# LiuZhu-CV/PAIF

Hardware: AMD Instinct MI355X
Metric: fused image-pairs/sec at 480x640 bs=8 per GPU (fusion-net forward) (higher is better)
Workload: dtype f16 (IEEE fp16 maps and conv weights, one fp16 MFMA per product, f32 accumulate; stems, guided filter and the last map fp32)

## Files before the change

paif_amd/csrc/conv_dma.h:

```cpp
#pragma once
#include <hip/hip_runtime.h>

namespace paif_conv_dma {

struct Args {
  const void* src[3];
  const void* res[3];
  const void* wpk;
  const float* scale;
  const float* shift;
  const float* prelu;
  void* out;
  float alpha;
  int nsrc, nres, act, kh;
  int cout;
  int B, H, W, reverse;
  float* cpool;
  int f16;
  int dil;
  int in_relu;
  int out_f32;
};

bool eligible(int nsrc, int nres, int B, int H, int W, float alpha);
bool eligible16(int nsrc, int nres, int B, int H, int W, float alpha);
bool eligible7(int nsrc, int nres, int B, int H, int W, float alpha);
bool eligible_d2(int nsrc, int nres, int B, int H, int W, float alpha);
bool can_cpool(int nsrc, int nres, int kh, int cout, int dil);
int launch(const Args& a, hipStream_t st);

bool eligible_1x1(int nsrc, int nres, int B, int H, int W);
int launch_1x1(const Args& a, hipStream_t st);

bool eligible_rows(int nsrc, int nres, int in_relu, int cpool, int f16, int out_f32, int B, int H, int W);
int launch_rows(const Args& a, hipStream_t st);

}
```

paif_amd/csrc/conv_mfma.hip:

```cpp
#include <stdlib.h>

#include "conv_dma.h"
#include "paif_common.h"
#include <type_traits>

#ifndef PAIF_UB_HOOKS
#define PAIF_UB_HOOKS 3
#endif
#ifndef PAIF_UB
#define PAIF_UB 11
#endif

namespace {

typedef float f32x16 __attribute__((ext_vector_type(16)));

#ifndef PAIF_TH
#define PAIF_TH 8
#endif
constexpr int TH = PAIF_TH;
constexpr int TW = 32;
constexpr int NTHREADS = 256;
constexpr int SEGS_PER_WAVE = TH / 4;

// ... 1292 lines not shown
  } else {
    const int t = tid - 4 * 64;
    const int q = t & 7, px = t >> 3;
    const float4 sc = *reinterpret_cast<const float4*>((a.scale ? a.scale : k_ones) + 4 * q);
    const float4 sh = *reinterpret_cast<const float4*>((a.shift ? a.shift : k_zeros) + 4 * q);
    const float slope = *(a.act == 1 ? a.prelu : k_zeros);
    const int nres = a.res[0] ? (a.res[1] ? (a.res[2] ? 3 : 2) : 1) : 0;
    const unsigned lane_off = (unsigned)px * 32u + 4u * (unsigned)q;
    auto run = [&](auto nres_c) {
      constexpr int NR = decltype(nres_c)::value;
      float4 r[NR > 0 ? NR : 1][8];
      auto request = [&](int i) {
        int b, y0, x0;
        tile_of(min(i, cnt - 1), b, y0, x0);
        const size_t base = ((size_t)(b * a.H + y0) * a.W + x0) * 32;
        const unsigned lo = x0 + px < a.W ? lane_off : 0u;
#pragma unroll
        for (int k = 0; k < NR; ++k)
#pragma unroll
          for (int j = 0; j < 8; ++j) {
            const int yy = min(y0 + j, a.H - 1) - y0;
            r[k][j] = paif::ldq_nt<BFR>(a.res[k], base + (size_t)yy * a.W * 32 + lo);
          }
      };
      if (cnt > 0) request(0);
      int s2 = 0, i2 = 0;
      for (int g = 0; g <= S + 1; ++g) {
        if (g >= 2) {
          if (s2 == nsrc - 1) {
            int b, y0, x0;
            tile_of(i2, b, y0, x0);
            float4 o[8];
#pragma unroll
            for (int j = 0; j < 8; ++j) o[j] = *reinterpret_cast<const float4*>(outbuf + (j * 32 + px) * 32 + 4 * q);
            const size_t base = ((size_t)(b * a.H + y0) * a.W + x0) * 32;
            const bool colok = x0 + px < a.W;
#pragma unroll
            for (int j = 0; j < 8; ++j) {
              float4 v = o[j];
              v.x = v.x * sc.x + sh.x; v.y = v.y * sc.y + sh.y; v.z = v.z * sc.z + sh.z; v.w = v.w * sc.w + sh.w;
              if (a.act == 1) {
                v.x = paif::prelu_f(v.x, slope); v.y = paif::prelu_f(v.y, slope);
                v.z = paif::prelu_f(v.z, slope); v.w = paif::prelu_f(v.w, slope);
              } else if (a.act == 2) {
                v.x = fmaxf(v.x, 0.f); v.y = fmaxf(v.y, 0.f); v.z = fmaxf(v.z, 0.f); v.w = fmaxf(v.w, 0.f);
              }
              v.x *= a.alpha; v.y *= a.alpha; v.z *= a.alpha; v.w *= a.alpha;
#pragma unroll
              for (int k = 0; k < NR; ++k) { v.x += r[k][j].x; v.y += r[k][j].y; v.z += r[k][j].z; v.w += r[k][j].w; }
              if (colok && y0 + j < a.H)
                paif::stq_nt<BFO>(a.out, base + (size_t)j * a.W * 32 + lane_off, v);
              if (a.cpool) {
                float mx = fmaxf(fmaxf(v.x, v.y), fmaxf(v.z, v.w)), sm = (v.x + v.y) + (v.z + v.w);
                paif::pix8_max_sum(mx, sm);
                if (colok && y0 + j < a.H && q == 0)
                  *reinterpret_cast<float2*>(a.cpool + ((base + (size_t)j * a.W * 32) >> 5) * 4 + (size_t)px * 4) = make_float2(mx, sm * (1.0f / 32.0f));
              }
            }
            if (NR > 0) request(i2 + 1);
          }
          if (++s2 == nsrc) { s2 = 0; ++i2; }
        }
        lds_barrier();
        lds_barrier();
      }
    };
    if (nres == 0) run(std::integral_constant<int, 0>{});
    else if (nres == 1) run(std::integral_constant<int, 1>{});
    else if (nres == 2) run(std::integral_constant<int, 2>{});
    else run(std::integral_constant<int, 3>{});
  }
}

template <int KH, int DIL, int ST = 0>
__global__ __launch_bounds__(WS_THREADS, 1) void conv_bf16x3_ws(ConvArgs a, int ntiles) { conv_ws_body<KH, DIL, ST, false>(a, ntiles); }
template <int KH, int DIL, int ST = 0>
__global__ __launch_bounds__(WS_THREADS, 1) void conv_bf16x3_wsr(ConvArgs a, int ntiles) { conv_ws_body<KH, DIL, ST, true>(a, ntiles); }

template <int KH, int DIL, int ST = 0>
int launch_bf16x3_ws(const ConvArgs& a, hipStream_t st) {
  constexpr int P = DIL * (KH - 1) / 2;
  constexpr size_t lds_bytes = 2 * (size_t)(TH + 2 * P) * (TW + 2 * P) * 144 + 8 * 32 * 32 * 4;
  static_assert(lds_bytes <= 160 * 1024, "two tile buffers + the parked tile do not fit LDS");
  static bool raised = false;
  constexpr bool HAS_RELU = KH == 3 && DIL == 2 && paif::st_in(ST) != 0 && paif::st_low(ST) != 7;
  if (!raised) {
    hipError_t e = hipFuncSetAttribute(reinterpret_cast<const void*>(&conv_bf16x3_ws<KH, DIL, ST>),
                                       hipFuncAttributeMaxDynamicSharedMemorySize, (int)lds_bytes);
    if constexpr (HAS_RELU) {
      if (e == hipSuccess)
        e = hipFuncSetAttribute(reinterpret_cast<const void*>(&conv_bf16x3_wsr<KH, DIL, ST>), hipFuncAttributeMaxDynamicSharedMemorySize,
                                (int)lds_bytes);
    }
    if (e != hipSuccess) {
      paif::set_error("conv2d(bf16x3 ws): cannot raise dynamic LDS to %zu: %s", lds_bytes, hipGetErrorString(e));
      return (int)e;
    }
    raised = true;
  }
  if (a.in_act == 2) {
    if constexpr (HAS_RELU) {
      hipLaunchKernelGGL((conv_bf16x3_wsr<KH, DIL, ST>), dim3(256), dim3(WS_THREADS), lds_bytes, st, a, a.nblk);
      PAIF_LAUNCH_CHECK("conv2d(bf16x3 wsr)");
      return 0;
    }
    paif::set_error("conv2d(bf16x3 ws): input ReLU is built for the bf16-stored dilation-2 3x3 only");
    return PAIF_ENOSUP;
  }
  hipLaunchKernelGGL((conv_bf16x3_ws<KH, DIL, ST>), dim3(256), dim3(WS_THREADS), lds_bytes, st, a, a.nblk);
  PAIF_LAUNCH_CHECK("conv2d(bf16x3 ws)");
  return 0;
}

static inline bool ws_enabled() {
  static const bool on = [] {
    const char* e = getenv("PAIF_CONV_WS");
    return !(e && e[0] == '0');
  }();
  return on;
}
static inline bool st_h16(const ConvArgs& a) { return a.st == 1 || a.st == 3; }
static inline bool st_is_f16(const ConvArgs& a) { return a.st >= 3; }
static inline bool ws_eligible(const ConvArgs& a) {
  return ws_enabled() && a.nblk >= 1024 && !a.pool_partial && a.cout == 32 && (a.in_act == 0 || (a.in_act == 2 && st_h16(a))) &&
         (size_t)a.H * a.W * 128 < ((size_t)1 << 32);
}

static inline bool res_eligible(const ConvArgs& a) {
  static const bool on = [] {
    const char* e = getenv("PAIF_CONV_RES");
    return !(e && e[0] == '0');
  }();
  static const int ms_res = [] {
    const char* e = getenv("PAIF_CONV_RES_NSRC");
    return e ? atoi(e) : 1;
  }();
  return on && !st_is_f16(a) && (a.nsrc == 1 || (a.wl0 && a.st == 1 && a.in_act == 0 && a.nsrc <= ms_res)) && a.nblk >= 2048 && a.cout == 32 && a.in_act <= 2 && (PAIF_RES_ROWS == 8 || !a.pool_partial) &&
         (size_t)a.B * a.H * a.W * 128 < ((size_t)1 << 31);
}

static inline bool needs_hooks(const ConvArgs& a) { return a.in_act >= 3 || a.aux_out || a.epi_dact; }

static inline bool takes_ws(const ConvArgs& a, int kh, int dil) {
#if PAIF_TH == 8
  if (needs_hooks(a) || kh > 3 || !ws_eligible(a)) return false;
  if (a.st == 4) return dil == 2 && a.nsrc == 1 && a.in_act == 0;
  if (kh == 1) return !a.res[0] && a.in_act == 0;
  return dil == 2 && a.nsrc == 1 && st_h16(a);
#else
  return false;
#endif
}

enum ConvVariant { CV_PLAIN, CV_HOOKS, CV_WS, CV_RES, CV_MS, CV_DMA, CV_ROWS };
static inline int res_count(const ConvArgs& a) { return a.res[0] ? (a.res[1] ? (a.res[2] ? 3 : 2) : 1) : 0; }
static inline ConvVariant bf16x3_variant(const ConvArgs& a, int kh, int dil) {
  if (needs_hooks(a)) return CV_HOOKS;
  if (dil == 1 && st_h16(a) && a.wl0 && a.in_act == 0 && !a.pool_partial &&
      ((kh == 3 && a.cout == 32 && paif_conv_dma::eligible(a.nsrc, res_count(a), a.B, a.H, a.W, a.alpha)) ||
       (kh == 3 && a.cout == 16 && paif_conv_dma::eligible16(a.nsrc, res_count(a), a.B, a.H, a.W, a.alpha)) ||
       (kh == 7 && a.cout == 32 && paif_conv_dma::eligible7(a.nsrc, res_count(a), a.B, a.H, a.W, a.alpha))))
    return CV_DMA;
  if (kh == 3 && dil == 2 && (st_h16(a) || a.st == 4) && a.wl0 && a.in_act == 0 && !a.pool_partial && !a.cpool && a.cout == 32 &&
      paif_conv_dma::eligible_rows(a.nsrc, res_count(a), 0, 0, st_is_f16(a) ? 1 : 0, a.st == 4 ? 1 : 0, a.B, a.H, a.W))
    return CV_ROWS;
  if (kh == 3 && dil == 2 && st_h16(a) && a.wl0 && a.in_act == 2 && !a.pool_partial && a.cout == 32 &&
      paif_conv_dma::eligible_d2(a.nsrc, res_count(a), a.B, a.H, a.W, a.alpha))
    return CV_DMA;
  if (kh == 1 && dil == 1 && st_h16(a) && a.wl0 && a.in_act == 0 && !a.pool_partial && a.cout == 32 && ws_eligible(a) &&
      paif_conv_dma::eligible_1x1(a.nsrc, res_count(a), a.B, a.H, a.W))
    return CV_DMA;
  if (takes_ws(a, kh, dil)) return CV_WS;
  if (kh == 3 && dil == 1 && !st_is_f16(a)) {
    if (res_eligible(a)) return CV_RES;
    if (ms_enabled() && a.nsrc >= 2 && a.cout == 32 && a.in_act == 0 && !a.pool_partial &&
        (size_t)a.B * a.H * a.W * 128 < ((size_t)1 << 32))
      return CV_MS;
  }
  return CV_PLAIN;
}

static inline bool variant_can_cpool(const ConvArgs& a, int kh, int dil) {
  if (a.cout != 32 || needs_hooks(a)) return false;
  if (bf16x3_variant(a, kh, dil) == CV_DMA) return paif_conv_dma::can_cpool(a.nsrc, res_count(a), kh, a.cout, dil);
  return true;
}

template <int KH, int DIL, int ST>
int launch_bf16x3_st(const ConvArgs& a, hipStream_t st) {
  const ConvVariant cv = bf16x3_variant(a, KH, DIL);
  switch (cv) {
    case CV_ROWS:
    case CV_DMA: {
      paif_conv_dma::Args d{};
      for (int s = 0; s < 3; ++s) { d.src[s] = a.src[s]; d.res[s] = a.res[s]; }
      d.wpk = a.wpk; d.scale = a.scale; d.shift = a.shift; d.prelu = a.prelu; d.out = a.out; d.alpha = a.alpha;
      d.nsrc = a.nsrc; d.nres = res_count(a); d.act = a.act; d.B = a.B; d.H = a.H; d.W = a.W; d.reverse = a.reverse; d.kh = KH; d.cout = a.cout;
      d.f16 = paif::st_f16(ST) ? 1 : 0;
      d.cpool = a.cpool;
      d.dil = DIL; d.in_relu = a.in_act == 2 ? 1 : 0;
      d.out_f32 = paif::st_out(ST) == 0 ? 1 : 0;
      return cv == CV_ROWS ? paif_conv_dma::launch_rows(d, st) : paif_conv_dma::launch(d, st);
    }
    case CV_HOOKS:
      if constexpr (ST == 0) return launch_bf16x3_h<KH, DIL, true>(a, st);
      paif::set_error("conv2d: the gradient hooks (in_act >= 3, aux_out, epi_dact) are built for fp32 storage only");
      return PAIF_ENOSUP;
    case CV_WS:
#if PAIF_TH == 8
      if constexpr (KH <= 3) return launch_bf16x3_ws<KH, DIL, ST>(a, st);
#endif
      break;
    case CV_RES:
      if constexpr (KH == 3 && DIL == 1 && !paif::st_f16(ST)) {
        if constexpr (ST == 4) {
          if (a.nsrc == 2) return launch_bf16x3_res<3, 1, 2, ST>(a, st);
          if (a.nsrc == 3) return launch_bf16x3_res<3, 1, 3, ST>(a, st);
        }
        return launch_bf16x3_res<3, 1, 1, ST>(a, st);
      }
      break;
    case CV_MS:
      if constexpr (KH == 3 && DIL == 1 && !paif::st_f16(ST)) return a.nsrc == 2 ? launch_bf16x3_ms<3, 1, 2, ST>(a, st) : launch_bf16x3_ms<3, 1, 3, ST>(a, st);
      break;
    default: break;
  }
  return launch_bf16x3_h<KH, DIL, false, ST>(a, st);
}

static inline int kernel_st(const ConvArgs& a) {
  if (a.st == 4) return 15;
  const int st = a.st == 3 ? 1 : a.st;
  const int base = st == 1 ? (a.in_act == 1 ? 3 : 1) : st;
  const int code = (a.wl0 && base) ? base + 3 : base;
  return a.st >= 3 ? code + 8 : code;
}

template <int KH, int DIL>
int launch_bf16x6(const ConvArgs& a, hipStream_t st) {
  if (a.st != 0) {
    paif::set_error("conv2d: precision bf16x6 is built for fp32-stored maps");
    return PAIF_ENOSUP;
  }
  return needs_hooks(a) ? launch_bf16x3_h<KH, DIL, true, 0, 3>(a, st) : launch_bf16x3_h<KH, DIL, false, 0, 3>(a, st);
}

template <int KH, int DIL>
int launch_f16x3(const ConvArgs& a, hipStream_t st) {
  if (a.st != 0) {
    paif::set_error("conv2d: precision f16x3 is built for fp32-stored maps");
    return PAIF_ENOSUP;
  }
  return needs_hooks(a) ? launch_bf16x3_h<KH, DIL, true, 0, 2, 1>(a, st) : launch_bf16x3_h<KH, DIL, false, 0, 2, 1>(a, st);
}

template <int KH, int DIL>
int launch_bf16x3(const ConvArgs& a, hipStream_t st) {
  const int code = kernel_st(a);
  if (code == 0) return launch_bf16x3_st<KH, DIL, 0>(a, st);
  if constexpr ((KH == 1 || KH == 3 || KH == 7) && (DIL == 1 || (KH == 3 && DIL == 2))) {
    switch (code) {
      case 1: return launch_bf16x3_st<KH, DIL, 1>(a, st);
      case 3: return launch_bf16x3_st<KH, DIL, 3>(a, st);
      case 4: return launch_bf16x3_st<KH, DIL, 4>(a, st);
      case 6: return launch_bf16x3_st<KH, DIL, 6>(a, st);
      default: break;
    }
    if constexpr (KH == 1) {
      if (code == 2) return launch_bf16x3_st<KH, DIL, 2>(a, st);
      if (code == 5) return launch_bf16x3_st<KH, DIL, 5>(a, st);
    }
    switch (code) {
      case 12: return launch_bf16x3_st<KH, DIL, 12>(a, st);
      case 14: return launch_bf16x3_st<KH, DIL, 14>(a, st);
      default: break;
    }
    if constexpr (KH == 1) {
      if (code == 9) return launch_bf16x3_st<KH, DIL, 9>(a, st);
    }
    if constexpr (KH == 3 && DIL == 2) {
      if (code == 15) return launch_bf16x3_st<KH, DIL, 15>(a, st);
    }
  }
  paif::set_error("conv2d: storage %d is not built for the %dx%d dilation-%d kernel", a.st, KH, KH, DIL);
  return PAIF_ENOSUP;
}

__global__ void pack_weight_bf16x3_kernel(const float* __restrict__ w, unsigned short* __restrict__ wpk, int cout, int nsrc,
                                          int kh) {
  const int ntap = kh * kh;
  const int total = nsrc * ntap * 2 * 2 * 64 * 8;
  for (int idx = blockIdx.x * blockDim.x + threadIdx.x; idx < total; idx += gridDim.x * blockDim.x) {
    const int j = idx & 7, lane = (idx >> 3) & 63, part = (idx >> 9) & 1, ks = (idx >> 10) & 1;
    int rest = idx >> 11;
    const int tap = rest % ntap;
    const int s = rest / ntap;
    const int n = lane & 31, hh = lane >> 5;
    const int c = s * 32 + 16 * ks + 8 * hh + j;
    const float v = (n < cout) ? w[((size_t)n * (nsrc * 32) + c) * ntap + tap] : 0.f;
    const __bf16 hi = (__bf16)v;
    const __bf16 out = part == 0 ? hi : (__bf16)(v - (float)hi);
    wpk[idx] = __builtin_bit_cast(unsigned short, out);
  }
}

__global__ void compose_dw_pw_kernel(const float* __restrict__ dw, const float* __restrict__ pw, float* __restrict__ out, int cout,
                                     int cin, int ntap) {
  const int total = cout * cin * ntap;
  for (int idx = blockIdx.x * blockDim.x + threadIdx.x; idx < total; idx += gridDim.x * blockDim.x) {
    const int tap = idx % ntap, ci = (idx / ntap) % cin, co = idx / (ntap * cin);
    out[idx] = pw[co * cin + ci] * dw[ci * ntap + tap];
  }
}

__global__ void compose_pw_conv_kernel(const float* __restrict__ pw, const float* __restrict__ w, float* __restrict__ out, int cout, int cmid,
                                       int cin, int ntap) {
  const int total = cout * cin * ntap;
  for (int idx = blockIdx.x * blockDim.x + threadIdx.x; idx < total; idx += gridDim.x * blockDim.x) {
    const int rest = idx % (cin * ntap), co = idx / (cin * ntap);
    double acc = 0.0;
    for (int m = 0; m < cmid; ++m) acc = fma((double)pw[co * cmid + m], (double)w[(size_t)m * cin * ntap + rest], acc);
    out[idx] = (float)acc;
  }
}

__device__ __forceinline__ unsigned short bf16x6_piece(float v, int part) {
  const __bf16 hi = (__bf16)v;
  const float r1 = v - (float)hi;
  const __bf16 mid = (__bf16)r1;
  const __bf16 out = part == 0 ? hi : (part == 1 ? mid : (__bf16)(r1 - (float)mid));
  return __builtin_bit_cast(unsigned short, out);
}
__global__ void pack_weight_bf16x6_kernel(const float* __restrict__ w, unsigned short* __restrict__ wpk, int cout, int nsrc, int kh) {
  const int ntap = kh * kh;
  const int total = nsrc * ntap * 2 * 3 * 64 * 8;
  for (int idx = blockIdx.x * blockDim.x + threadIdx.x; idx < total; idx += gridDim.x * blockDim.x) {
    const int j = idx & 7, lane = (idx >> 3) & 63;
    int rest = idx >> 9;
    const int part = rest % 3; rest /= 3;
    const int ks = rest & 1; rest >>= 1;
    const int tap = rest % ntap;
    const int s = rest / ntap;
    const int n = lane & 31, hh = lane >> 5;
    const int c = s * 32 + 16 * ks + 8 * hh + j;
    const float v = (n < cout) ? w[((size_t)n * (nsrc * 32) + c) * ntap + tap] : 0.f;
    wpk[idx] = bf16x6_piece(v, part);
  }
}
__global__ void pack_decomp1x1_bf16x6_kernel(const float* __restrict__ w, unsigned short* __restrict__ wpk) {
  const int total = 3 * 2 * 3 * 64 * 8;
  for (int idx = blockIdx.x * blockDim.x + threadIdx.x; idx < total; idx += gridDim.x * blockDim.x) {
    const int j = idx & 7, lane = (idx >> 3) & 63;
    int rest = idx >> 9;
    const int part = rest % 3; rest /= 3;
// ... 45 lines not shown
    const float v = (n < cout) ? w[((size_t)n * (nsrc * 32) + c) * ntap + tap] : 0.f;
    wpk[idx] = f16x2_piece(v, part);
  }
}
__global__ void pack_decomp1x1_hf_f16x2_kernel(const float* __restrict__ w, unsigned short* __restrict__ wpk) {
  const int total = 3 * 2 * 2 * 64 * 8;
  for (int idx = blockIdx.x * blockDim.x + threadIdx.x; idx < total; idx += gridDim.x * blockDim.x) {
    const int j = idx & 7, lane = (idx >> 3) & 63, part = (idx >> 9) & 1, ks = (idx >> 10) & 1, s = idx >> 11;
    const int n = lane & 31, hh = lane >> 5;
    const int c = 16 * ks + 8 * hh + j;
    const float* wn = w + n * 128;
    float v;
    if (s == 0) v = wn[c] + wn[32 + c];
    else if (s == 1) v = wn[64 + c] - wn[c];
    else v = wn[96 + c] - wn[32 + c];
    wpk[idx] = f16x2_piece(v, part);
  }
}

template <int KH, int DIL, int CIN, bool HOOKS>
int launch_h(const ConvArgs& a, hipStream_t st) {
  constexpr int P = DIL * (KH - 1) / 2;
  constexpr size_t tile_bytes = (size_t)(TH + 2 * P) * (TW + 2 * P) * (CIN + 4) * 4;
  constexpr size_t epi_bytes = (size_t)TH * 32 * 32 * 4;
  constexpr size_t lds_bytes = tile_bytes > epi_bytes ? tile_bytes : epi_bytes;
  static_assert(lds_bytes <= 160 * 1024, "tile does not fit LDS");
  if (lds_bytes > 64 * 1024) {
    hipError_t e = hipFuncSetAttribute(reinterpret_cast<const void*>(&conv_mfma_f32<KH, DIL, CIN, HOOKS>),
                                       hipFuncAttributeMaxDynamicSharedMemorySize, (int)lds_bytes);
    if (e != hipSuccess) {
      paif::set_error("conv2d: cannot raise dynamic LDS to %zu: %s", lds_bytes, hipGetErrorString(e));
      return (int)e;
    }
  }
  hipLaunchKernelGGL((conv_mfma_f32<KH, DIL, CIN, HOOKS>), dim3(a.nblk), dim3(NTHREADS), lds_bytes, st, a);
  PAIF_LAUNCH_CHECK("conv2d");
  return 0;
}

template <int KH, int DIL, int CIN>
int launch(const ConvArgs& a, hipStream_t st) {
  return needs_hooks(a) ? launch_h<KH, DIL, CIN, true>(a, st) : launch_h<KH, DIL, CIN, false>(a, st);
}

__global__ void pack_weight_kernel(const float* __restrict__ w, float* __restrict__ wpk, int cout, int nsrc, int cin,
                                   int kh) {
  const int ntap = kh * kh, no = cin / 8;
  const int total = nsrc * ntap * no * 256;
  for (int idx = blockIdx.x * blockDim.x + threadIdx.x; idx < total; idx += gridDim.x * blockDim.x) {
    const int i = idx & 3, lane = (idx >> 2) & 63;
    int rest = idx >> 8;
    const int o = rest % no; rest /= no;
    const int tap = rest % ntap;
    const int s = rest / ntap;
    const int n = lane & 31, h = lane >> 5;
    const int c = s * cin + 8 * o + 4 * h + i;
    wpk[idx] = (n < cout) ? w[((size_t)n * (nsrc * cin) + c) * ntap + tap] : 0.f;
  }
}

__global__ void pack_decomp1x1_kernel(const float* __restrict__ w, float* __restrict__ wpk) {
  const int total = 3 * 4 * 256;
  for (int idx = blockIdx.x * blockDim.x + threadIdx.x; idx < total; idx += gridDim.x * blockDim.x) {
    const int i = idx & 3, lane = (idx >> 2) & 63;
    const int o = (idx >> 8) & 3, s = idx >> 10;
    const int n = lane & 31, h = lane >> 5;
    const int c = 8 * o + 4 * h + i;
    const float* wn = w + n * 128;
    float v;
    if (s == 0) v = wn[64 + c] + wn[96 + c];
    else if (s == 1) v = wn[c] - wn[64 + c];
    else v = wn[32 + c] - wn[96 + c];
    wpk[idx] = v;
  }
}

__global__ void bn_fold_kernel(const float* g, const float* bta, const float* mean, const float* var, float eps,
                               float* scale, float* shift, int C) {
  const int c = blockIdx.x * blockDim.x + threadIdx.x;
  if (c < C) {
    const float s = g[c] / sqrtf(var[c] + eps);
    scale[c] = s;
    shift[c] = bta[c] - mean[c] * s;
  }
}

}

extern "C" {

int paif_conv2d_blocks(int B, int H, int W) { return B * ((H + TH - 1) / TH) * ((W + TW - 1) / TW); }

size_t paif_conv_wpk_floats(int nsrc, int cin, int kh) { return (size_t)nsrc * kh * kh * (cin / 8) * 256; }

int paif_conv2d_is_persistent(const paif_conv_desc* d, int B, int H, int W) {
  if (!d || (d->precision != PAIF_CONV_BF16X3 && d->precision != PAIF_CONV_BF16 && d->precision != PAIF_CONV_F16 && d->precision != PAIF_CONV_F16X2) ||
      d->cin != 32 || B <= 0 || H <= 0 || W <= 0)
    return 0;
  ConvArgs a{};
  for (int s = 0; s < 3; ++s) a.res[s] = d->res[s];
  a.pool_partial = d->pool_partial; a.nsrc = d->nsrc; a.in_act = d->in_act; a.cout = d->cout;
  a.aux_out = d->aux_out; a.epi_dact = d->epi_dact; a.st = d->storage;
  a.H = H; a.W = W;
  a.nblk = B * ((W + TW - 1) / TW) * ((H + TH - 1) / TH);
  return takes_ws(a, d->kh, d->dil) ? 1 : 0;
}

int paif_conv2d_can_cpool(const paif_conv_desc* d, int B, int H, int W) {
  if (!d || d->cout != 32 || d->cin != 32 || B <= 0 || H <= 0 || W <= 0 || d->precision == PAIF_CONV_F32 || d->precision == PAIF_CONV_BF16X6 || d->precision == PAIF_CONV_F16X3) return 0;
  ConvArgs a{};
  for (int s = 0; s < 3; ++s) a.res[s] = d->res[s];
  a.pool_partial = d->pool_partial; a.nsrc = d->nsrc; a.in_act = d->in_act; a.cout = d->cout;
  a.aux_out = d->aux_out; a.epi_dact = d->epi_dact;
  a.B = B; a.H = H; a.W = W;
  a.nblk = B * ((W + TW - 1) / TW) * ((H + TH - 1) / TH);
  a.st = d->storage; a.wl0 = (d->precision == PAIF_CONV_BF16 || d->precision == PAIF_CONV_F16) ? 1 : 0; a.alpha = d->alpha;
  return variant_can_cpool(a, d->kh, d->dil) ? 1 : 0;
}

int paif_conv2d_kernel_name(const paif_conv_desc* d, int B, int H, int W, char* buf, int buflen) {
  PAIF_REQUIRE(d && buf && buflen > 0 && B > 0 && H > 0 && W > 0, PAIF_EINVAL, "conv2d_kernel_name: bad arguments");
  ConvArgs a{};
  for (int s = 0; s < 3; ++s) a.res[s] = d->res[s];
  a.pool_partial = d->pool_partial; a.nsrc = d->nsrc; a.in_act = d->in_act; a.cout = d->cout;
  a.aux_out = d->aux_out; a.epi_dact = d->epi_dact;
  a.B = B; a.H = H; a.W = W;
  a.nblk = B * ((W + TW - 1) / TW) * ((H + TH - 1) / TH);
  a.st = d->storage; a.wl0 = (d->precision == PAIF_CONV_BF16 || d->precision == PAIF_CONV_F16) ? 1 : 0; a.alpha = d->alpha;
  a.cpool = d->cpool;
  const int code = kernel_st(a);
  if (d->precision == PAIF_CONV_BF16X6 && d->cin == 32) {
    snprintf(buf, buflen, "conv_mfma_bf16x6<%d, %d, %s, 0>", d->kh, d->dil, needs_hooks(a) ? "true" : "false");
    return 0;
  }
  if (d->precision == PAIF_CONV_F16X3 && d->cin == 32) {
    snprintf(buf, buflen, "conv_mfma_f16x3<%d, %d, %s, 0>", d->kh, d->dil, needs_hooks(a) ? "true" : "false");
    return 0;
  }
  if (d->precision != PAIF_CONV_BF16X3 && d->precision != PAIF_CONV_BF16 && d->precision != PAIF_CONV_F16 && d->precision != PAIF_CONV_F16X2) {
    snprintf(buf, buflen, "conv_mfma_f32<%d, %d, %d, %s>", d->kh, d->dil, d->cin, needs_hooks(a) ? "true" : "false");
    return 0;
  }
  if (d->cin != 32) {
    snprintf(buf, buflen, "conv_mfma_f32<%d, %d, %d, %s>", d->kh, d->dil, d->cin, needs_hooks(a) ? "true" : "false");
    return 0;
  }
  switch (bf16x3_variant(a, d->kh, d->dil)) {
    case CV_DMA:
      if (d->kh == 7) snprintf(buf, buflen, "conv7x7_h16_dma<%d>", a.st >= 3 ? 2 : 1);
      else if (d->kh == 1) snprintf(buf, buflen, "conv_h16_dma_1x1<%d>", a.st >= 3 ? 2 : 1);
      else snprintf(buf, buflen, "conv3x3_h16_dma<%d, %d, %d, %s, %d, %d>", d->nsrc, res_count(a), a.st >= 3 ? 2 : 1, d->cpool ? "true" : "false",
                    d->dil, d->dil == 2 ? 2 : 0);
      break;
    case CV_ROWS: snprintf(buf, buflen, "conv3x3_h16_dma_rows<%d, %d, %s>", a.st >= 3 ? 2 : 1, res_count(a), a.st == 4 ? "true" : "false"); break;
    case CV_WS: snprintf(buf, buflen, "conv_bf16x3_ws%s<%d, %d, %d>", d->in_act == 2 ? "r" : "", d->kh, d->dil, code); break;
    case CV_RES: snprintf(buf, buflen, "conv_bf16x3_res<%d, %d, %d, %d, %d>", d->kh, d->dil, d->nsrc, PAIF_RES_ROWS, code); break;
    case CV_MS: snprintf(buf, buflen, "conv_bf16x3_ms<%d, %d, %d, %d>", d->kh, d->dil, d->nsrc, code); break;
    case CV_HOOKS: snprintf(buf, buflen, "conv_mfma_bf16x3<%d, %d, true, %d>", d->kh, d->dil, code); break;
    default: snprintf(buf, buflen, "conv_mfma_bf16x3<%d, %d, false, %d>", d->kh, d->dil, code); break;
  }
  return 0;
}

int paif_conv2d_fwd(const paif_conv_desc* d, int B, int H, int W, paif_stream_t stream) {
  PAIF_REQUIRE(d && d->out && d->wpk, PAIF_EINVAL, "conv2d: null descriptor/out/wpk");
  PAIF_REQUIRE(d->nsrc >= 1 && d->nsrc <= 3, PAIF_EINVAL, "conv2d: nsrc=%d", d->nsrc);
  for (int s = 0; s < d->nsrc; ++s) PAIF_REQUIRE(d->src[s], PAIF_EINVAL, "conv2d: src[%d] null", s);
  PAIF_REQUIRE(d->cout == 32 || d->cout == 16, PAIF_ENOSUP, "conv2d: cout=%d", d->cout);
  PAIF_REQUIRE(B > 0 && H > 0 && W > 0, PAIF_EINVAL, "conv2d: empty shape %dx%dx%d", B, H, W);
  PAIF_REQUIRE(d->in_act != 1 || d->in_prelu, PAIF_EINVAL, "conv2d: in_act=PReLU without slope");
  PAIF_REQUIRE(d->act != 1 || d->prelu, PAIF_EINVAL, "conv2d: act=PReLU without slope");
  ConvArgs a;
  for (int s = 0; s < 3; ++s) {
    a.src[s] = s < d->nsrc ? d->src[s] : nullptr;
    a.res[s] = d->res[s];
  }
  a.wpk = reinterpret_cast<const float4*>(d->wpk);
  a.in_prelu = d->in_prelu; a.scale = d->scale; a.shift = d->shift; a.prelu = d->prelu;
  a.out = d->out; a.pool_partial = d->pool_partial; a.cpool = d->cpool; a.alpha = d->alpha;
  a.nsrc = d->nsrc; a.in_act = d->in_act; a.act = d->act; a.cout = d->cout;
  a.aux_out = d->aux_out; a.in_aux = d->in_aux; a.in_scale = d->in_scale; a.in_alpha = d->in_alpha;
  a.epi_aux = d->epi_aux; a.epi_dact = d->epi_dact;
  PAIF_REQUIRE(d->in_act >= 0 && d->in_act <= 5, PAIF_EINVAL, "conv2d: in_act=%d", d->in_act);
  PAIF_REQUIRE(!(d->in_act == 3 || d->in_act == 4) || (d->in_aux && d->nsrc == 1), PAIF_EINVAL,
               "conv2d: in_act=%d needs in_aux and a single source", d->in_act);
  PAIF_REQUIRE(d->in_act != 3 || d->in_prelu, PAIF_EINVAL, "conv2d: in_act=3 without slope");
  PAIF_REQUIRE(d->epi_dact >= 0 && d->epi_dact <= 2 && (!d->epi_dact || d->epi_aux), PAIF_EINVAL, "conv2d: epi_dact=%d", d->epi_dact);
  PAIF_REQUIRE(d->epi_dact != 1 || d->prelu, PAIF_EINVAL, "conv2d: epi_dact=PReLU without slope");
  a.B = B; a.H = H; a.W = W;
  a.tilesX = (W + TW - 1) / TW; a.tilesY = (H + TH - 1) / TH; a.nblk = B * a.tilesX * a.tilesY;
  a.reverse = d->reverse_tiles ? 1 : 0;
  a.st = d->storage;
  a.wl0 = (d->precision == PAIF_CONV_BF16 || d->precision == PAIF_CONV_F16) ? 1 : 0;
  PAIF_REQUIRE(d->storage >= 0 && d->storage <= 4, PAIF_EINVAL, "conv2d: storage=%d", d->storage);
  const bool st_bf = d->storage == PAIF_ST_BF16 || d->storage == PAIF_ST_F32_BF16, st_hf = d->storage == PAIF_ST_F16 || d->storage == PAIF_ST_F16_F32;
  PAIF_REQUIRE(!st_bf || ((d->precision == PAIF_CONV_BF16X3 || d->precision == PAIF_CONV_BF16) && d->cin == 32), PAIF_ENOSUP,
               "conv2d: bf16 storage needs the split-bf16 kernels (cin 32)");
  PAIF_REQUIRE(!st_hf || ((d->precision == PAIF_CONV_F16 || d->precision == PAIF_CONV_F16X2) && d->cin == 32), PAIF_ENOSUP,
               "conv2d: fp16 storage takes precision F16 / F16X2 (cin 32)");
  PAIF_REQUIRE(d->precision != PAIF_CONV_BF16 || st_bf, PAIF_ENOSUP, "conv2d: precision bf16 is built for bf16-stored maps only");
  PAIF_REQUIRE((d->precision != PAIF_CONV_F16 && d->precision != PAIF_CONV_F16X2) || st_hf, PAIF_ENOSUP,
               "conv2d: precision fp16 is built for fp16-stored maps only");
  PAIF_REQUIRE(d->storage != PAIF_ST_F16_F32 || d->precision == PAIF_CONV_F16, PAIF_ENOSUP, "conv2d: fp16 in / fp32 out takes plain fp16 weights");
  hipStream_t st = paif::as_stream(stream);
  PAIF_REQUIRE(!d->cpool || paif_conv2d_can_cpool(d, B, H, W), PAIF_ENOSUP, "conv2d: no fused ChannelPool for this descriptor (paif_conv2d_can_cpool)");
  PAIF_REQUIRE(d->cin == 32 || d->cin == 16, PAIF_ENOSUP, "conv2d: cin=%d", d->cin);
  PAIF_REQUIRE(d->precision == PAIF_CONV_F32 || d->precision == PAIF_CONV_BF16X3 || d->precision == PAIF_CONV_BF16 ||
                   d->precision == PAIF_CONV_BF16X6 || d->precision == PAIF_CONV_F16 || d->precision == PAIF_CONV_F16X2 ||
                   d->precision == PAIF_CONV_F16X3, PAIF_EINVAL,
               "conv2d: precision=%d", d->precision);
  PAIF_REQUIRE((d->precision != PAIF_CONV_BF16X6 && d->precision != PAIF_CONV_F16X3) || d->cin == 32, PAIF_ENOSUP, "conv2d: bf16x6 / f16x3 need 32-channel sources");
  const int key = d->kh * 100 + d->dil * 10 + (d->cin == 32 ? 0 : 1);
  if (d->precision == PAIF_CONV_F16X3) {
    switch (key) {
      case 110: return launch_f16x3<1, 1>(a, st);
      case 310: return launch_f16x3<3, 1>(a, st);
      case 320: return launch_f16x3<3, 2>(a, st);
      case 510: return launch_f16x3<5, 1>(a, st);
      case 710: return launch_f16x3<7, 1>(a, st);
      default: break;
    }
    paif::set_error("conv2d(f16x3): kernel %dx%d dil %d cin %d not built", d->kh, d->kh, d->dil, d->cin);
    return PAIF_ENOSUP;
  }
  if (d->precision == PAIF_CONV_BF16X6) {
    switch (key) {
      case 110: return launch_bf16x6<1, 1>(a, st);
      case 310: return launch_bf16x6<3, 1>(a, st);
      case 320: return launch_bf16x6<3, 2>(a, st);
      case 510: return launch_bf16x6<5, 1>(a, st);
      case 710: return launch_bf16x6<7, 1>(a, st);
      default: break;
    }
    paif::set_error("conv2d(bf16x6): kernel %dx%d dil %d cin %d not built", d->kh, d->kh, d->dil, d->cin);
    return PAIF_ENOSUP;
  }
  if (d->precision == PAIF_CONV_BF16X3 || d->precision == PAIF_CONV_BF16 || d->precision == PAIF_CONV_F16 || d->precision == PAIF_CONV_F16X2) {
    switch (key) {
      case 110: return launch_bf16x3<1, 1>(a, st);
      case 310: return launch_bf16x3<3, 1>(a, st);
      case 320: return launch_bf16x3<3, 2>(a, st);
      case 510: return launch_bf16x3<5, 1>(a, st);
      case 520: return launch_bf16x3<5, 2>(a, st);
      case 710: return launch_bf16x3<7, 1>(a, st);
      case 720: return launch_bf16x3<7, 2>(a, st);
      default: break;
    }
    paif::set_error("conv2d(bf16x3): kernel %dx%d dil %d cin %d not built", d->kh, d->kh, d->dil, d->cin);
    return PAIF_ENOSUP;
  }
  switch (key) {
    case 110: return launch<1, 1, 32>(a, st);
    case 310: return launch<3, 1, 32>(a, st);
    case 320: return launch<3, 2, 32>(a, st);
    case 510: return launch<5, 1, 32>(a, st);
    case 520: return launch<5, 2, 32>(a, st);
    case 710: return launch<7, 1, 32>(a, st);
    case 720: return launch<7, 2, 32>(a, st);
    case 311: return launch<3, 1, 16>(a, st);
    default: break;
  }
  paif::set_error("conv2d: kernel %dx%d dil %d cin %d not built", d->kh, d->kh, d->dil, d->cin);
  return PAIF_ENOSUP;
}

int paif_pack_conv_weight_bf16x3(const float* w, float* wpk, int cout, int nsrc, int kh, paif_stream_t stream) {
  PAIF_REQUIRE(w && wpk, PAIF_EINVAL, "pack_conv_weight_bf16x3: null pointer");
  PAIF_REQUIRE(cout >= 1 && cout <= 32 && nsrc >= 1 && nsrc <= 3 && kh >= 1 && kh <= 7, PAIF_ENOSUP,
               "pack_conv_weight_bf16x3: cout=%d nsrc=%d kh=%d", cout, nsrc, kh);
  const int total = nsrc * kh * kh * 2048;
  hipLaunchKernelGGL(pack_weight_bf16x3_kernel, dim3((total + 255) / 256), dim3(256), 0, paif::as_stream(stream), w,
                     reinterpret_cast<unsigned short*>(wpk), cout, nsrc, kh);
  PAIF_LAUNCH_CHECK("pack_conv_weight_bf16x3");
  return 0;
}

int paif_pack_conv_weight_f16x2(const float* w, float* wpk, int cout, int nsrc, int kh, paif_stream_t stream) {
  PAIF_REQUIRE(w && wpk, PAIF_EINVAL, "pack_conv_weight_f16x2: null pointer");
  PAIF_REQUIRE(cout >= 1 && cout <= 32 && nsrc >= 1 && nsrc <= 3 && kh >= 1 && kh <= 7, PAIF_ENOSUP,
               "pack_conv_weight_f16x2: cout=%d nsrc=%d kh=%d", cout, nsrc, kh);
  const int total = nsrc * kh * kh * 2048;
  hipLaunchKernelGGL(pack_weight_f16x2_kernel, dim3((total + 255) / 256), dim3(256), 0, paif::as_stream(stream), w,
                     reinterpret_cast<unsigned short*>(wpk), cout, nsrc, kh);
  PAIF_LAUNCH_CHECK("pack_conv_weight_f16x2");
  return 0;
}

int paif_pack_decomp1x1_hf_weight_f16x2(const float* w, float* wpk, paif_stream_t stream) {
  PAIF_REQUIRE(w && wpk, PAIF_EINVAL, "pack_decomp1x1_hf_weight_f16x2: null pointer");
  hipLaunchKernelGGL(pack_decomp1x1_hf_f16x2_kernel, dim3(24), dim3(256), 0, paif::as_stream(stream), w,
                     reinterpret_cast<unsigned short*>(wpk));
  PAIF_LAUNCH_CHECK("pack_decomp1x1_hf_weight_f16x2");
  return 0;
}

int paif_pack_conv_weight_bf16x6(const float* w, float* wpk, int cout, int nsrc, int kh, paif_stream_t stream) {
  PAIF_REQUIRE(w && wpk, PAIF_EINVAL, "pack_conv_weight_bf16x6: null pointer");
  PAIF_REQUIRE(cout >= 1 && cout <= 32 && nsrc >= 1 && nsrc <= 3 && kh >= 1 && kh <= 7, PAIF_ENOSUP,
               "pack_conv_weight_bf16x6: cout=%d nsrc=%d kh=%d", cout, nsrc, kh);
  const int total = nsrc * kh * kh * 3072;
  hipLaunchKernelGGL(pack_weight_bf16x6_kernel, dim3((total + 255) / 256), dim3(256), 0, paif::as_stream(stream), w,
                     reinterpret_cast<unsigned short*>(wpk), cout, nsrc, kh);
  PAIF_LAUNCH_CHECK("pack_conv_weight_bf16x6");
  return 0;
}

// ... 61 lines not shown
```

Measured before the change: 2614.

## Add row-streaming DMA kernel for single-source dilation-1 3x3 fp16 convs

Adds a new 3x3, dilation-1, 32->32 conv kernel in which each wave walks a vertical strip of 32 columns row by row. Input rows are loaded by buffer-to-LDS DMA into a five-slot ring that prefetches two rows ahead, and the weights stay in registers for the whole run. Each output row reuses the two input rows already held from the previous step instead of reloading a full halo tile, and the epilogue goes through a small LDS parking area before vector stores. Dispatch now picks this path ahead of the existing tiled DMA kernel whenever the map is large enough. Uncovered cases, such as fp32 output, could be routed here and then be refused at launch.

```diff
diff --git a/paif_amd/csrc/conv_dma.h b/paif_amd/csrc/conv_dma.h
--- a/paif_amd/csrc/conv_dma.h
+++ b/paif_amd/csrc/conv_dma.h
@@ -35,4 +35,7 @@
 bool eligible_rows(int nsrc, int nres, int in_relu, int cpool, int f16, int out_f32, int B, int H, int W);
 int launch_rows(const Args& a, hipStream_t st);
 
+bool eligible_rows_d1(int nsrc, int nres, int B, int H, int W, float alpha);
+int launch_rows_d1(const Args& a, hipStream_t st);
+
 }
diff --git a/paif_amd/csrc/conv_dma_rows_d1.hip b/paif_amd/csrc/conv_dma_rows_d1.hip
--- /dev/null
+++ b/paif_amd/csrc/conv_dma_rows_d1.hip
@@ -0,0 +1,251 @@
+#include <stdint.h>
+#include <stdlib.h>
+
+#include <type_traits>
+
+#include "conv_dma.h"
+#include "paif_common.h"
+
+namespace paif_conv_dma {
+namespace {
+
+typedef float f32x16 __attribute__((ext_vector_type(16)));
+typedef unsigned u32x4 __attribute__((ext_vector_type(4)));
+
+constexpr int RW = 32;
+constexpr int RWH = RW + 2;
+constexpr int DPS = 3;
+constexpr int SLOT = DPS * 1024;
+constexpr int NSLOT = 5, PF = NSLOT - 3;
+constexpr int PARK = 32 * 32 * 4;
+constexpr int WAVE_LDS = NSLOT * SLOT + PARK;
+constexpr int WAVES = 4;
+constexpr int LDS_BYTES = WAVES * WAVE_LDS;
+constexpr int MAX_WAVES = 2048;
+constexpr int MIN_RUN = 16;
+constexpr int N_ROW = PF * DPS;
+static_assert(2 * LDS_BYTES <= 160 * 1024, "two workgroups per CU do not fit LDS");
+static_assert(RWH * 4 <= DPS * 64, "DMA instructions do not cover the row piece");
+constexpr unsigned RSRC_W3 = 0x00020000u;
+constexpr unsigned OOB = 0x80000000u;
+
+#ifndef CR1_LD_AUX
+#define CR1_LD_AUX 2
+#endif
+#ifndef CR1_ST_AUX
+#define CR1_ST_AUX 0
+#endif
+#define CR1_VMWAIT(n) asm volatile("s_waitcnt vmcnt(%0)" ::"n"(n) : "memory")
+#define CR1_RD128(dst, addr, off) asm volatile("ds_read_b128 %0, %1 offset:%2" : "=v"(dst) : "v"(addr), "n"(off) : "memory")
+#define CR1_WR32(addr, val, off) asm volatile("ds_write_b32 %0, %1 offset:%2" ::"v"(addr), "v"(val), "n"(off) : "memory")
+#define CR1_LGKM(n, g) asm volatile("s_waitcnt lgkmcnt(" #n ")" : "+v"(A[(g) % 3][0]), "+v"(A[(g) % 3][1]), "+v"(A[(g) % 3][2])::"memory")
+
+__device__ __forceinline__ void dma16(__amdgpu_buffer_rsrc_t rsrc, unsigned voff, unsigned lds_off) {
+  __builtin_amdgcn_raw_ptr_buffer_load_lds(rsrc, (__attribute__((address_space(3))) void*)(uintptr_t)lds_off, 16, voff, 0, 0, CR1_LD_AUX);
+}
+
+template <int F>
+__global__ __launch_bounds__(WAVES * 64, 2) void conv3x3_h16_dma_rows_d1(Args a, int total, int SX, int run) {
+  __shared__ __attribute__((aligned(16))) unsigned char smem[LDS_BYTES];
+  asm volatile("" ::"v"((unsigned)(uintptr_t)(__attribute__((address_space(3))) unsigned char*)smem) : "memory");
+
+  const int tid = threadIdx.x, l = tid & 63;
+  const int w = __builtin_amdgcn_readfirstlane(tid >> 6);
+  const int p = l & 31, hh = l >> 5;
+  const int gw = blockIdx.x * WAVES + w;
+  int pos = gw * run;
+  const int end = min(total, pos + run);
+  if (pos >= end) return;
+  const int H = a.H, W = a.W;
+
+  const int map_bytes = a.B * H * W * 64;
+  const __amdgpu_buffer_rsrc_t rs_src = __builtin_amdgcn_make_buffer_rsrc(const_cast<void*>(a.src[0]), 0, map_bytes, RSRC_W3);
+  const __amdgpu_buffer_rsrc_t rs_out = __builtin_amdgcn_make_buffer_rsrc(a.out, 0, map_bytes, RSRC_W3);
+
+  u32x4 bw[9][2];
+  {
+    const __amdgpu_buffer_rsrc_t rs_w = __builtin_amdgcn_make_buffer_rsrc(const_cast<void*>(a.wpk), 0, 9 * 2 * 2 * 1024, RSRC_W3);
+#pragma unroll
+    for (int tap = 0; tap < 9; ++tap)
+#pragma unroll
+      for (int ks = 0; ks < 2; ++ks) bw[tap][ks] = __builtin_amdgcn_raw_buffer_load_b128(rs_w, (unsigned)l * 16u, ((tap * 2 + ks) * 2) * 1024, 0);
+  }
+  float esc[8], esh[8];
+#pragma unroll
+  for (int j = 0; j < 8; ++j) {
+    const int c = 8 * (l & 3) + j;
+    esc[j] = (a.scale ? a.scale[c] : 1.f) * a.alpha;
+    esh[j] = (a.shift ? a.shift[c] : 0.f) * a.alpha;
+  }
+  const float e_slope = a.act == 1 ? *a.prelu : (a.act == 2 ? 0.f : 1.f);
+
+  int d_col[DPS];
+  unsigned d_rel[DPS];
+#pragma unroll
+  for (int i = 0; i < DPS; ++i) {
+    const int n = 64 * i + l, c = n >> 2;
+    d_col[i] = c;
+    d_rel[i] = (unsigned)(c * 64 + (((n & 3) ^ ((c >> 2) & 3)) * 16));
+  }
+  const unsigned lds_w = (unsigned)(w * WAVE_LDS);
+  unsigned a_rd[3][2];
+#pragma unroll
+  for (int dx = 0; dx < 3; ++dx)
+#pragma unroll
+    for (int ks = 0; ks < 2; ++ks) {
+      const int c = p + dx;
+      a_rd[dx][ks] = lds_w + (unsigned)(c * 64 + (((2 * ks + hh) ^ ((c >> 2) & 3)) * 16));
+    }
+  const unsigned a_pw = lds_w + NSLOT * SLOT + (unsigned)((4 * hh * 32 + p) * 4);
+  const unsigned a_pr = lds_w + NSLOT * SLOT + (unsigned)((l >> 2) * 128 + (l & 3) * 32);
+  const unsigned e_lane = (unsigned)l * 16u;
+
+  f32x16 acc;
+
+  while (pos < end) {
+    const int q = pos / H, i0 = pos - q * H;
+    const int n = min(H - i0, end - pos);
+    const int b = q / SX, x0 = (q - b * SX) * RW;
+    pos += n;
+    bool colok[DPS];
+#pragma unroll
+    for (int i = 0; i < DPS; ++i) colok[i] = d_col[i] < RWH && (unsigned)(x0 - 1 + d_col[i]) < (unsigned)W;
+    const bool xok0 = x0 + (l >> 2) < W, xok1 = x0 + 16 + (l >> 2) < W;
+    auto issue_row = [&](int m, int slot) {
+      const int j = i0 - 1 + m;
+      const unsigned dead = (j >= 0 && j < H && m <= n + 1) ? 0u : OOB;
+      const unsigned rowb = (unsigned)((b * H + j) * W + x0 - 1) * 64u;
+#pragma unroll
+      for (int i = 0; i < DPS; ++i) dma16(rs_src, (colok[i] ? rowb + d_rel[i] : OOB) | dead, lds_w + (unsigned)(slot * SLOT + i * 1024));
+    };
+
+    int cur = 0;
+    auto step = [&](int t) {
+      const int s1 = cur + 1 >= NSLOT ? cur + 1 - NSLOT : cur + 1, s2 = cur + 2 >= NSLOT ? cur + 2 - NSLOT : cur + 2;
+      const int fill = cur == 0 ? NSLOT - 1 : cur - 1;
+      issue_row(t + 2 + PF, fill);
+      CR1_VMWAIT(N_ROW);
+      const unsigned rb[3] = {(unsigned)(cur * SLOT), (unsigned)(s1 * SLOT), (unsigned)(s2 * SLOT)};
+      u32x4 A[3][3];
+      auto read = [&](int gi) {
+        const int ks = gi / 3, dx = gi % 3;
+#pragma unroll
+        for (int dy = 0; dy < 3; ++dy) {
+          const unsigned ad = a_rd[dx][ks] + rb[dy];
+          CR1_RD128(A[gi % 3][dy], ad, 0);
+        }
+      };
+      auto mma = [&](auto gitag) {
+        constexpr int gi = decltype(gitag)::value, ks = gi / 3, dx = gi % 3;
+        __builtin_amdgcn_sched_barrier(0);
+#pragma unroll
+        for (int dy = 0; dy < 3; ++dy) {
+          if (gi == 0 && dy == 0) {
+            const f32x16 z = {0.f, 0.f, 0.f, 0.f, 0.f, 0.f, 0.f, 0.f, 0.f, 0.f, 0.f, 0.f, 0.f, 0.f, 0.f, 0.f};
+            acc = paif::mfma16<F>(A[gi % 3][dy], bw[dy * 3 + dx][ks], z);
+          } else {
+            acc = paif::mfma16<F>(A[gi % 3][dy], bw[dy * 3 + dx][ks], acc);
+          }
+        }
+        __builtin_amdgcn_sched_barrier(0);
+      };
+      typedef std::integral_constant<int, 0> G0;
+      typedef std::integral_constant<int, 1> G1;
+      typedef std::integral_constant<int, 2> G2;
+      typedef std::integral_constant<int, 3> G3;
+      typedef std::integral_constant<int, 4> G4;
+      typedef std::integral_constant<int, 5> G5;
+      read(0);
+      read(1);
+      read(2);
+      CR1_LGKM(6, 0); mma(G0{}); read(3);
+      CR1_LGKM(6, 1); mma(G1{}); read(4);
+      CR1_LGKM(6, 2); mma(G2{}); read(5);
+      CR1_LGKM(6, 3); mma(G3{});
+      CR1_LGKM(3, 4); mma(G4{});
+      CR1_LGKM(0, 5); mma(G5{});
+
+      asm volatile("s_nop 15\n\ts_nop 7" ::: "memory");
+#pragma unroll
+      for (int r = 0; r < 16; ++r) {
+        const float v = acc[r];
+        CR1_WR32(a_pw, v, ((r & 3) + 8 * (r >> 2)) * 128);
+      }
+      u32x4 tq[2][2];
+      CR1_RD128(tq[0][0], a_pr, 0);
+      CR1_RD128(tq[0][1], a_pr, 16);
+      CR1_RD128(tq[1][0], a_pr, 2048);
+      CR1_RD128(tq[1][1], a_pr, 2048 + 16);
+      asm volatile("s_waitcnt lgkmcnt(0)" : "+v"(tq[0][0]), "+v"(tq[0][1]), "+v"(tq[1][0]), "+v"(tq[1][1])::"memory");
+      __builtin_amdgcn_sched_barrier(0);
+      const unsigned orow = (unsigned)((b * H + i0 + t) * W + x0) * 64u;
+#pragma unroll
+      for (int it = 0; it < 2; ++it) {
+        float ev[8];
+#pragma unroll
+        for (int j = 0; j < 8; ++j) {
+          const float v = __builtin_fmaf(__uint_as_float(tq[it][j >> 2][j & 3]), esc[j], esh[j]);
+          ev[j] = __builtin_fmaf(e_slope, fminf(v, 0.f), fmaxf(v, 0.f));
+        }
+        const uint2 h0 = paif::f32_to_h4<F>(make_float4(ev[0], ev[1], ev[2], ev[3]));
+        const uint2 h1 = paif::f32_to_h4<F>(make_float4(ev[4], ev[5], ev[6], ev[7]));
+        u32x4 od = {h0.x, h0.y, h1.x, h1.y};
+        __builtin_amdgcn_raw_buffer_store_b128(od, rs_out, (it ? xok1 : xok0) ? orow + (unsigned)(it * 1024) + e_lane : OOB, 0, CR1_ST_AUX);
+        asm volatile("s_nop 2" : "+v"(od));
+      }
+      __builtin_amdgcn_sched_barrier(0);
+      cur = s1;
+    };
+
+#pragma unroll
+    for (int m = 0; m < 2 + PF; ++m) issue_row(m, m);
+    for (int t = 0; t < n; ++t) step(t);
+    CR1_VMWAIT(0);
+  }
+}
+
+int env_rows_d1() {
+  const char* d = getenv("PAIF_CONV_DMA");
+  if (d && d[0] == '0') return 0;
+  const char* e = getenv("PAIF_CONV_DMA_ROWS_D1");
+  if (!e || !e[0]) return -1;
+  return e[0] == '0' ? 0 : 1;
+}
+
+template <int F>
+void launch_rows_d1_f(const Args& a, hipStream_t st) {
+  const int SX = (a.W + RW - 1) / RW;
+  const int total = a.B * SX * a.H;
+  const int per = (total + MAX_WAVES - 1) / MAX_WAVES;
+  const int run = per > MIN_RUN ? per : MIN_RUN;
+  const int waves = (total + run - 1) / run;
+  hipLaunchKernelGGL((conv3x3_h16_dma_rows_d1<F>), dim3((waves + WAVES - 1) / WAVES), dim3(WAVES * 64), 0, st, a, total, SX, run);
+}
+
+}
+
+bool eligible_rows_d1(int nsrc, int nres, int B, int H, int W, float alpha) {
+  const int sw = env_rows_d1();
+  if (sw == 0 || nsrc != 1 || nres != 0 || !(alpha > 0.f)) return false;
+  if ((long long)B * H * W * 64 >= (1ll << 31)) return false;
+  if (sw == 1) return true;
+  return H >= 64 && (long long)B * H * ((W + RW - 1) / RW) >= (long long)MIN_RUN * MAX_WAVES;
+}
+
+int launch_rows_d1(const Args& a, hipStream_t st) {
+  if (a.nsrc != 1 || a.nres != 0 || a.cout != 32 || a.cpool || a.in_relu || a.dil != 1 || a.kh != 3 || a.out_f32 || !(a.alpha > 0.f) ||
+      (long long)a.B * a.H * a.W * 64 >= (1ll << 31)) {
+    paif::set_error("conv2d(h16 dma rows d1): built for one source, dilation 1, 32 -> 32, no residual map, no input activation, no ChannelPool");
+    return PAIF_ENOSUP;
+  }
+  if (a.f16) launch_rows_d1_f<2>(a, st);
+  else launch_rows_d1_f<1>(a, st);
+  hipError_t e = hipGetLastError();
+  if (e != hipSuccess) {
+    paif::set_error("conv2d(h16 dma rows d1): launch failed: %s", hipGetErrorString(e));
+    return (int)e;
+  }
+  return 0;
+}
+
+}
diff --git a/paif_amd/csrc/conv_mfma.hip b/paif_amd/csrc/conv_mfma.hip
--- a/paif_amd/csrc/conv_mfma.hip
+++ b/paif_amd/csrc/conv_mfma.hip
@@ -1468,10 +1468,13 @@
 #endif
 }
 
-enum ConvVariant { CV_PLAIN, CV_HOOKS, CV_WS, CV_RES, CV_MS, CV_DMA, CV_ROWS };
+enum ConvVariant { CV_PLAIN, CV_HOOKS, CV_WS, CV_RES, CV_MS, CV_DMA, CV_ROWS, CV_ROWS_D1 };
 static inline int res_count(const ConvArgs& a) { return a.res[0] ? (a.res[1] ? (a.res[2] ? 3 : 2) : 1) : 0; }
 static inline ConvVariant bf16x3_variant(const ConvArgs& a, int kh, int dil) {
   if (needs_hooks(a)) return CV_HOOKS;
+  if (kh == 3 && dil == 1 && st_h16(a) && a.wl0 && a.in_act == 0 && !a.pool_partial && !a.cpool && a.cout == 32 &&
+      paif_conv_dma::eligible_rows_d1(a.nsrc, res_count(a), a.B, a.H, a.W, a.alpha))
+    return CV_ROWS_D1;
   if (dil == 1 && st_h16(a) && a.wl0 && a.in_act == 0 && !a.pool_partial &&
       ((kh == 3 && a.cout == 32 && paif_conv_dma::eligible(a.nsrc, res_count(a), a.B, a.H, a.W, a.alpha)) ||
        (kh == 3 && a.cout == 16 && paif_conv_dma::eligible16(a.nsrc, res_count(a), a.B, a.H, a.W, a.alpha)) ||
@@ -1498,7 +1501,8 @@
 
 static inline bool variant_can_cpool(const ConvArgs& a, int kh, int dil) {
   if (a.cout != 32 || needs_hooks(a)) return false;
-  if (bf16x3_variant(a, kh, dil) == CV_DMA) return paif_conv_dma::can_cpool(a.nsrc, res_count(a), kh, a.cout, dil);
+  const ConvVariant cv = bf16x3_variant(a, kh, dil);
+  if (cv == CV_DMA || cv == CV_ROWS_D1) return paif_conv_dma::can_cpool(a.nsrc, res_count(a), kh, a.cout, dil);
   return true;
 }
 
@@ -1507,6 +1511,7 @@
   const ConvVariant cv = bf16x3_variant(a, KH, DIL);
   switch (cv) {
     case CV_ROWS:
+    case CV_ROWS_D1:
     case CV_DMA: {
       paif_conv_dma::Args d{};
       for (int s = 0; s < 3; ++s) { d.src[s] = a.src[s]; d.res[s] = a.res[s]; }
@@ -1516,6 +1521,7 @@
       d.cpool = a.cpool;
       d.dil = DIL; d.in_relu = a.in_act == 2 ? 1 : 0;
       d.out_f32 = paif::st_out(ST) == 0 ? 1 : 0;
+      if (cv == CV_ROWS_D1) return paif_conv_dma::launch_rows_d1(d, st);
       return cv == CV_ROWS ? paif_conv_dma::launch_rows(d, st) : paif_conv_dma::launch(d, st);
     }
     case CV_HOOKS:
@@ -1867,6 +1873,7 @@
       else snprintf(buf, buflen, "conv3x3_h16_dma<%d, %d, %d, %s, %d, %d>", d->nsrc, res_count(a), a.st >= 3 ? 2 : 1, d->cpool ? "true" : "false",
                     d->dil, d->dil == 2 ? 2 : 0);
       break;
+    case CV_ROWS_D1: snprintf(buf, buflen, "conv3x3_h16_dma_rows_d1<%d>", a.st >= 3 ? 2 : 1); break;
     case CV_ROWS: snprintf(buf, buflen, "conv3x3_h16_dma_rows<%d, %d, %s>", a.st >= 3 ? 2 : 1, res_count(a), a.st == 4 ? "true" : "false"); break;
     case CV_WS: snprintf(buf, buflen, "conv_bf16x3_ws%s<%d, %d, %d>", d->in_act == 2 ? "r" : "", d->kh, d->dil, code); break;
     case CV_RES: snprintf(buf, buflen, "conv_bf16x3_res<%d, %d, %d, %d, %d>", d->kh, d->dil, d->nsrc, PAIF_RES_ROWS, code); break;
```

Result: no change. 2637 (median of 6 runs) (+0.9%).
